# e4s2024/E4S2024

Hardware: AMD Instinct MI355X
Metric: 1024x1024 faces/sec (StyleGAN2 regional synthesis, gen_img) (higher is better)
Workload: dtype f16+mxfp6x2 (masked 3x3 layers >= 32^2) / bf16x3 (all other layers); 1 GPU; BASELINE configs[1]: StyleGAN2 1024x1024 synthesis from random W+, 12-region masks, batch=4/GPU; batch_per_gpu=4, global_batch=4, parallelism=frames x1, streams_per_gpu=2

## Files before the change

### e4s2024_amd/_lib.py

```python
from __future__ import annotations

import ctypes
import os
import re

HERE = os.path.dirname(os.path.abspath(__file__))
SO_PATH = os.environ.get("E4S_HIP_LIB") or os.path.join(HERE, "lib", "libe4s_hip.so")
HEADER = os.path.join(os.path.dirname(HERE), "include", "e4s_hip.h")

c_int, c_i64, c_f32, c_ptr = ctypes.c_int, ctypes.c_int64, ctypes.c_float, ctypes.c_void_p

_SCALARS = {"int": c_int, "int64_t": c_i64, "float": c_f32, "unsigned": ctypes.c_uint}
_RETURNS = {"int": c_int, "const char*": ctypes.c_char_p}


def _ctype(decl: str, where: str):
    if "*" in decl:
        return c_ptr
    ty = " ".join(decl.split()[:-1])
    if ty not in _SCALARS:
        raise TypeError(f"{where}: no ctypes rule for '{' '.join(decl.split())}' (known: pointers, {', '.join(_SCALARS)})")
    return _SCALARS[ty]


# ... 14 lines not shown
    for ret, name, args in re.findall(r"E4S_API\s+([\w\s*]+?)\s*\b(e4s_\w+)\s*\(([^()]*)\)\s*;", code):
        ret = " ".join(ret.split())
        if ret not in _RETURNS:
            raise TypeError(f"{name}: no ctypes rule for the return type '{ret}' (known: {', '.join(_RETURNS)})")
        restypes[name] = _RETURNS[ret]
        args = [] if args.strip() in ("", "void") else args.split(",")
        protos[name] = [_ctype(a, f"{name}: argument {i}") for i, a in enumerate(args)]
    if len(protos) != len(re.findall(r"\bE4S_API\b", code)):
        raise TypeError(f"the header has {len(re.findall('E4S_API', code))} E4S_API declarations, {len(protos)} were understood")
    return protos, restypes, structs, defines


with open(HEADER) as _f:
    _PROTOS, _RESTYPES, _STRUCTS, _DEFINES = parse_header(_f.read())

ABI_VERSION, ERR_ARG, MAX_REGIONS, LABEL_NONE, MAX_STYLE_JOBS, MAX_TARGETS, X_NHWC, OUT_NHWC, X_SP, OUT_SP = (_DEFINES["E4S_" + n] for n in (
    "ABI_VERSION", "ERR_ARG", "MAX_REGIONS", "LABEL_NONE", "MAX_STYLE_JOBS", "MAX_TARGETS", "X_NHWC", "OUT_NHWC", "X_SP", "OUT_SP"))


def targets(ptrs, weights):
    k = len(ptrs)
    if not 1 <= k <= MAX_TARGETS or len(weights) != k:
        raise ValueError(f"1 .. {MAX_TARGETS} targets with one weight each, got {k} targets and {len(weights)} weights")
    return (c_ptr * k)(*ptrs), (c_f32 * k)(*[float(w) for w in weights]), k


def declared_symbols():
    return list(_PROTOS)


class StyleJob(ctypes.Structure):
    _fields_ = _STRUCTS["E4sStyleJob"]
# ... 43 lines not shown
```

### e4s2024_amd/csrc/modconv_mx4.hip

```cpp
#include "modconv_mx_tile.h"

namespace {

constexpr int Q_TN = 64;
constexpr int Q_W1B = 3 * 2 * Q_TN * 16;
constexpr int Q_F6LO = 2 * 2 * Q_TN * 16;
constexpr int Q_F6HI = 2 * 2 * Q_TN * 8;
constexpr int Q_SCB = 1024;
constexpr int Q_PARB = Q_W1B + Q_F6LO + Q_F6HI + Q_SCB;
constexpr int Q_ROWB = 4 * Q_PARB;
constexpr int Q_NPIECE = Q_ROWB / 1024;
using CQ = SbCfg<2, 1, 1, 8, 5>;
constexpr int Q_PSTRIDE = 352;
constexpr int Q_PATCHB = 4 * Q_PSTRIDE * 16;
constexpr int Q_SSB = E4S_MAX_REGIONS * CKS * 4;
constexpr int Q_PATCH0 = 2 * Q_ROWB, Q_SS0 = Q_PATCH0 + 2 * Q_PATCHB, Q_LDS = Q_SS0 + 2 * Q_SSB;
static_assert(Q_LDS + 16 <= 160 * 1024 && (E4S_MAX_REGIONS + 1) * Q_TN * 4 <= Q_ROWB, "LDS plan");

#define Q_FENCE() do { asm volatile("" ::: "memory"); __builtin_amdgcn_sched_barrier(0); } while (0)

__global__ __launch_bounds__(256) void prep_weights_mx4_kernel(unsigned char* __restrict__ dst, const float* __restrict__ weight, const float* __restrict__ blur,
                                                               int cout, int cin, float scale) {
    const int nchunk = (cin + CKS - 1) / CKS;
    const int ntile = (cout + Q_TN - 1) / Q_TN;
// ... 265 lines not shown
    } else {
        c = l % G;
        item = l / G;
    }
    const int ntile = p.tiles_x * p.tiles_y;
    const int tile = (int)(item % (unsigned)ntile), b = (int)(item / (unsigned)ntile);
    const int y0 = (tile / p.tiles_x) * CQ::TH, x0 = (tile % p.tiles_x) * CQ::TW;
    int c_own;
    const bool uni = quad_uniform_tile(p, b, y0, x0, (int)(threadIdx.x >> 6), (int)(threadIdx.x & 31), c_own, reinterpret_cast<volatile int*>(lds_raw + Q_LDS));
    if (uni) {
        if (phase) return;
        q_tile_body(p, lds_raw, tile, (int)c, b, c_own);
    } else {
        SbParams pc = p;
        pc.wmx = reinterpret_cast<const unsigned char*>(p.whi);
        mx_tile_body<1, false, false, false>(pc, lds_raw, tile, (int)(2u * phase + (c & 1u)), 0, (int)(c >> 1), b);
    }
}

}

extern "C" int e4s_modconv_mx4_weight_bytes(int cout, int cin, int64_t* bytes) {
    E4S_REQUIRE(bytes && cout >= 1 && cin >= 1, "modconv_mx4_weight_bytes: bad arguments");
    *bytes = (int64_t)cdiv(cin, CKS) * cdiv(cout, Q_TN) * 3 * Q_ROWB;
    return 0;
}

extern "C" int e4s_modconv_prep_weights_mx4(void* dst, const float* weight, const float* blur, int cout, int cin, void* stream) {
    E4S_REQUIRE(dst && weight && blur, "modconv_prep_weights_mx4: null tensor");
    E4S_REQUIRE(cout >= 1 && cin >= 1, "modconv_prep_weights_mx4: bad size");
    E4S_REQUIRE(((uintptr_t)dst & 15) == 0, "modconv_prep_weights_mx4: the destination must be 16-byte aligned");
// ... 40 lines not shown
```

### e4s2024_amd/csrc/modconv_mx_tile.h

```cpp
#pragma once
#include <stdlib.h>

#include "common.h"
#include "sb_common.h"
#include "modconv_sb.h"

using namespace e4s;

#ifndef MX_ABL
#define MX_ABL 0
#endif

namespace {


typedef _Float16 f16x8 __attribute__((ext_vector_type(8)));
typedef _Float16 f16x2 __attribute__((ext_vector_type(2)));
typedef _Float16 f16x32 __attribute__((ext_vector_type(32)));
typedef unsigned u32x16 __attribute__((ext_vector_type(16)));
typedef unsigned u32x6 __attribute__((ext_vector_type(6)));
typedef int i32x8 __attribute__((ext_vector_type(8)));

constexpr int MX_TN = 128;
constexpr int MX_ROWB0 = 2 * 3 * 2 * MX_TN * 16;
// ... 78 lines not shown
struct MxLds {
    static constexpr int ROWB = ARITH ? MX_ROWB1 : MX_ROWB0;
    static constexpr int RING = 3 * ROWB;
    static constexpr int PATCH0 = RING;
    static constexpr int SS0 = PATCH0 + 2 * MX_PATCHB;
    static constexpr int BYTES = SS0 + 2 * MX_SSB;
    static constexpr int NPIECE = ROWB / 1024;
    static_assert(ROWB % 1024 == 0 && BYTES <= 160 * 1024, "LDS plan");
    static_assert((E4S_MAX_REGIONS + 5) * MX_TN * 4 + 64 <= RING, "the epilogue's tables overlay the weight ring");
};

constexpr int MX_NORM_MAX_CIN = 1024;
constexpr int MX_NORM_BYTES = 2 * MX_NORM_MAX_CIN * 4;
static_assert(MxLds<0>::BYTES + MX_NORM_BYTES <= 160 * 1024 && MxLds<1>::BYTES + MX_NORM_BYTES <= 160 * 1024, "LDS plan of the plain-convolution mode");

template <int ARITH, bool RGB, bool OSP, bool ENC = false>
__device__ __forceinline__ void mx_tile_body(const SbParams& p, unsigned char* lds_raw, const int tile, const int par, const int ks, const int cotile, const int b) {
    static_assert(!ENC || (!RGB && !OSP), "plain-convolution mode has its own epilogue");
    using L = MxLds<ARITH>;

    const int tid = threadIdx.x;
    const int lane = tid & 63;
    const int wave = __builtin_amdgcn_readfirstlane(tid >> 6) & 7;
    const int l5 = lane & 31, khalf = lane >> 5;

    const int pa = par >> 1, pb_ = par & 1;
    const int y0 = (tile / p.tiles_x) * C::TH, x0 = (tile % p.tiles_x) * C::TW;
    const int co0 = cotile * MX_TN;
    const int hw = p.h * p.w;
    const int ho = p.up ? 2 * p.h : p.h, wo = p.up ? 2 * p.w : p.w;
    const int nchunk = (p.cin + CKS - 1) / CKS;
// ... 344 lines not shown
                    if (co0 + n < p.cout) op[(size_t)(co0 + n) * hw] = v;
                }
        }
        return;
    }
    if (p.ksplit > 1) {
        float* part = p.partial + ((size_t)ks * p.bs + b) * p.cout * ho * wo;
        const int y = y0 + wave, x = x0 + l5;
        if (y < p.h && x < p.w) {
            const size_t opix = (size_t)(p.up ? 2 * y + pa : y) * wo + (p.up ? 2 * x + pb_ : x);
#pragma unroll
            for (int i = 0; i < 4; ++i)
#pragma unroll
                for (int r = 0; r < 16; ++r) {
                    const int co = co0 + i * 32 + (r & 3) + 8 * (r >> 2) + 4 * khalf;
                    if (co < p.cout) part[(size_t)co * ho * wo + opix] = acc[i][0][r];
                }
        }
        return;
    }
    if constexpr (MX_ABL & 1024) { if (acc[0][0][0] == 12345.f) p.out[tid] = acc[1][0][1] + acc[2][0][2] + acc[3][0][3]; return; }
    sb_epilogue<C, 4, 1, 8, RGB, OSP>(p, lds_raw, acc, cls, co0, b, y0, x0, pa, pb_, ho, wo, ub_skip);
}

}
```

### e4s2024_amd/csrc/modconv_sb.h

```cpp
#pragma once
#include "common.h"
#include "sb_common.h"

namespace e4s {

struct SbParams {
    float* out;
    const float* x;
    const uint4* whi;
    const uint4* wlo;
    const float* s;
    const float* d;
    const uint8_t* labels;
    const float* noise;
    const float* noise_weight;
    const float* act_bias;
    int lh, lw;
    float lscale_y, lscale_x;
    int noise_bstride;
    int act;
    int bs, cin, cout, h, w, nreg, up;
    int x_nhwc, out_nhwc;
    int tiles_x, tiles_y;
    int ksplit, chunks_per;
// ... 3 lines not shown
    const float* rgb_s;
    const float* rgb_bias;
    const float* rgb_skip;
    const float* rgb_upk;
    const float* s_next;
    int64_t plane_out;
    const uint8_t* uni_blocks;
    const int* uni_ctrl;
    const unsigned char* wmx;
    const float* in_mean;
    const float* in_rstd;
    const float* slope;
    int xcd_remap;
    int* flags;
    unsigned perm_mul;
};

template <int CB, int PB, int WC, int WP, int LOG_TW>
struct SbCfg {
    static constexpr int TN = WC * CB * 32;
    static constexpr int NPB = WP * PB;
    static constexpr int TW = 1 << LOG_TW;
    static constexpr int RPB = 32 >> LOG_TW;
    static constexpr int BPR = TW > 32 ? TW / 32 : 1;
    static constexpr int TH = TW > 32 ? NPB / BPR : NPB * RPB;
    static_assert(TW <= 32 || NPB % BPR == 0, "whole rows only");
    __host__ __device__ static constexpr int blk_y(int pbk, int l5) { return TW > 32 ? pbk / BPR : pbk * RPB + (l5 >> LOG_TW); }
    __host__ __device__ static constexpr int blk_x(int pbk, int l5) { return TW > 32 ? (pbk % BPR) * 32 + l5 : (l5 & (TW - 1)); }
    static constexpr int PW = TW + 2, PH = TH + 2;
    static constexpr int PATCH = PH * PW;
// ... 200 lines not shown
#pragma unroll
            for (int q = 0; q < PB; ++q) {
                const int pbk = wp * PB + q;
                const int y = y0 + C::blk_y(pbk, l5), x = x0 + C::blk_x(pbk, l5);
                if (y < p.h && x < p.w) {
                    const size_t opix = (size_t)y * wo + x;
#pragma unroll
                    for (int o = 0; o < 3; ++o)
                        p.rgb_out[((size_t)b * 3 + o) * ho * wo + opix] = rgbp[q][o] + xch[o * (C::NPB * 32) + pbk * 32 + l5] + rgbadd[q][o];
                }
            }
        }
    }
}

int launch_modconv_mx(SbParams& p, int arith, hipStream_t st, float* workspace, int64_t workspace_floats, bool plain_conv = false);

}
```

### e4s2024_amd/csrc/modconv_sb.hip

```cpp
#include <stdlib.h>

#include "common.h"
#include "sb_common.h"
#include "modconv_sb.h"

using namespace e4s;

__global__ __launch_bounds__(256) void prep_weights_sb_kernel(uint16_t* __restrict__ whi, uint16_t* __restrict__ wlo,
                                                              const float* __restrict__ weight, const float* __restrict__ blur, int cout,
                                                              int cin, int up, float scale) {
    const int npar = up ? 4 : 1;
    const int nchunk = (cin + CKS - 1) / CKS;
    const int64_t total = (int64_t)npar * nchunk * 9 * 2 * cout * 8;
    for (int64_t i = (int64_t)blockIdx.x * 256 + threadIdx.x; i < total; i += (int64_t)gridDim.x * 256) {
        const int e = (int)(i & 7);
        int64_t r = i >> 3;
        const int co = (int)(r % cout); r /= cout;
        const int half = (int)(r & 1); r >>= 1;
        const int tap = (int)(r % 9); r /= 9;
        const int chunk = (int)(r % nchunk);
        const int par = (int)(r / nchunk);
        const int ci = chunk * CKS + half * 8 + e;
        float v = 0.f;
        if (ci < cin) {
// ... 331 lines not shown
    }

    if (p.ksplit > 1) {
        float* part = p.partial + ((size_t)ks * p.bs + b) * p.cout * ho * wo;
#pragma unroll
        for (int q = 0; q < PB; ++q) {
            const int pbk = wp * PB + q;
            const int y = y0 + C::blk_y(pbk, l5), x = x0 + C::blk_x(pbk, l5);
            if (y >= p.h || x >= p.w) continue;
            const size_t opix = (size_t)(p.up ? 2 * y + pa : y) * wo + (p.up ? 2 * x + pb_ : x);
#pragma unroll
            for (int i = 0; i < CB; ++i)
#pragma unroll
                for (int r = 0; r < 16; ++r) {
                    const int co = co0 + (wc * CB + i) * 32 + (r & 3) + 8 * (r >> 2) + 4 * khalf;
                    if (co < p.cout) part[(size_t)co * ho * wo + opix] = acc[i][q][r];
                }
        }
        return;
    }

    E4S_PROF_MARK(g_prof_sb, 3);
    sb_epilogue<C, CB, PB, WP, RGB, OSP>(p, lds_raw, acc, cls, co0, b, y0, x0, pa, pb_, ho, wo, ub_skip);
    E4S_PROF_MARK(g_prof_sb, 4);
    E4S_PROF_DRAIN();
    E4S_PROF_MARK(g_prof_sb, 5);
}

__global__ __launch_bounds__(256) void modconv_sb_finalize_kernel(const SbParams p, int ho, int wo) {
    const size_t ohw = (size_t)ho * wo;
    const size_t per_b = (size_t)p.cout * ohw;
    const size_t total = (size_t)p.bs * per_b;
    const float nw = p.noise ? p.noise_weight[0] : 0.f;
    for (size_t i = (size_t)blockIdx.x * 256 + threadIdx.x; i < total; i += (size_t)gridDim.x * 256) {
        const int b = (int)(i / per_b);
        const size_t r = i - (size_t)b * per_b;
        const int co = (int)(r / ohw);
        const size_t opix = r - (size_t)co * ohw;
        const int oy = (int)(opix / wo), ox = (int)(opix - (size_t)oy * wo);
        float a = 0.f;
        for (int k = 0; k < p.ksplit; ++k) a += p.partial[(size_t)k * total + i];
        int c = 0;
        if (p.labels) c = p.labels[((size_t)b * p.lh + nearest_src(oy, p.lscale_y, p.lh)) * p.lw + nearest_src(ox, p.lscale_x, p.lw)];
        float v = 0.f;
        if (c < p.nreg) v = a * (p.d ? p.d[((size_t)b * p.nreg + c) * p.cout + co] : 1.f);
        if (p.noise) v += nw * p.noise[(size_t)b * p.noise_bstride + opix];
        if (p.act_bias) v += p.act_bias[co];
        if (p.act) v = (v > 0.f ? v : v * 0.2f) * 1.41421356237309515f;
        p.out[i] = v;
    }
}

template <int CB, int PB, int WC, int WP, int LOG_TW>
static int launch_sb_tconv(SbParams& p, hipStream_t st) {
    using C = SbCfg<CB, PB, WC, WP, LOG_TW>;
    p.tiles_x = cdiv(p.w + 1, C::TW);
    p.tiles_y = cdiv(p.h + 1, C::TH);
    p.up = 0;
    p.ksplit = 1;
    p.chunks_per = cdiv(p.cin, CKS);
    p.partial = nullptr;
    dim3 grid(p.tiles_x * p.tiles_y, cdiv(p.cout, C::TN), p.bs);
    hipLaunchKernelGGL((region_modconv_sb_kernel<CB, PB, WC, WP, LOG_TW, 2, true, true>), grid, dim3(C::NT), C::LDS_BYTES, st, p);
    return check_launch("modconv_tconv_sb");
// ... 57 lines not shown
    constexpr bool BIG = C::LDS_BYTES > 64 * 1024;
    constexpr int BIGW = C::NT / 256;
    if constexpr (BIG) {
        if (p.x_nhwc) return fail(E4S_ERR_ARG, "region_modconv3x3_sb: channels-last input is built for the single-region layers only");
        static const hipError_t attr = hipFuncSetAttribute(reinterpret_cast<const void*>(&region_modconv_sb_kernel<CB, PB, WC, WP, LOG_TW, BIGW, false, false>),
                                                           hipFuncAttributeMaxDynamicSharedMemorySize, C::LDS_BYTES);
        if (attr != hipSuccess) return fail((int)attr, "region_modconv3x3_sb: cannot raise the dynamic LDS limit: %s", hipGetErrorString(attr));
        hipLaunchKernelGGL((region_modconv_sb_kernel<CB, PB, WC, WP, LOG_TW, BIGW, false, false>), grid, dim3(C::NT), C::LDS_BYTES, st, p);
    } else if (p.x_nhwc) {
        if (p.labels || p.nreg != 1) return fail(E4S_ERR_ARG, "region_modconv3x3_sb: channels-last input is built for the single-region layers only");
        hipLaunchKernelGGL((region_modconv_sb_kernel<CB, PB, WC, WP, LOG_TW, 2, true, false, false, true>), grid, dim3(C::NT), uni_lds, st, p);
    } else if (!p.labels && p.nreg == 1)
        hipLaunchKernelGGL((region_modconv_sb_kernel<CB, PB, WC, WP, LOG_TW, 2, true, false>), grid, dim3(C::NT), uni_lds, st, p);
    else
        hipLaunchKernelGGL((region_modconv_sb_kernel<CB, PB, WC, WP, LOG_TW, 2, false, false>), grid, dim3(C::NT), C::LDS_BYTES, st, p);
    if (ksplit > 1) {
        const int g = (int)(cdiv64(out_floats, 256) < 2048 ? cdiv64(out_floats, 256) : 2048);
        hipLaunchKernelGGL(modconv_sb_finalize_kernel, dim3(g), dim3(256), 0, st, p, ho, wo);
    }
    return check_launch("region_modconv3x3_sb");
}

static inline bool layout_in_out_nhwc(int layout) { return (layout & (E4S_X_NHWC | E4S_OUT_NHWC)) != 0; }

static int region_modconv3x3_sb_impl(float* out, const float* x, const uint16_t* whi, const uint16_t* wlo, const float* s, const float* d,
                                     const uint8_t* labels, int lh, int lw, const float* noise, int noise_bs, const float* noise_weight,
                                     const float* act_bias, int act, int bs, int cin, int cout, int h, int w, int nreg, int up,
                                     float* workspace, int64_t workspace_floats, float* rgb_out, const float* rgb_wt, const float* rgb_s,
                                     const float* rgb_bias, const float* rgb_skip, const float* rgb_up_kernel, const float* s_next,
                                     const uint8_t* uniform_blocks, const int* uniform_ctrl, const void* wmx, int arith, int* flags, void* stream) {
    const int layout = up & (E4S_X_NHWC | E4S_OUT_NHWC | E4S_OUT_SP);
    up &= 1;
    const bool empty = bs == 0;
    E4S_REQUIRE(!(layout & E4S_OUT_SP) || (((s_next && rgb_out && out) || empty) && cout % 8 == 0 && !(layout & E4S_OUT_NHWC) && ((uintptr_t)out & 15) == 0),
                "region_modconv3x3_sb: split-plane output needs s_next, the fused ToRGB, cout %% 8 == 0 and a 16-byte aligned tensor");
    E4S_REQUIRE((((out || rgb_out) && x && s) || empty) && ((whi && wlo) || wmx), "region_modconv3x3_sb: null tensor");
    E4S_REQUIRE(!rgb_out || (rgb_wt && rgb_s && rgb_bias && (!rgb_skip || rgb_up_kernel) && w >= 32 && !up), "region_modconv3x3_sb: incomplete fused-ToRGB arguments");
    E4S_REQUIRE(bs >= 0 && cin >= 1 && cout >= 1 && h >= 1 && w >= 1, "region_modconv3x3_sb: bad size");
    E4S_REQUIRE(nreg >= 1 && nreg <= E4S_MAX_REGIONS, "region_modconv3x3_sb: %d regions (max %d)", nreg, E4S_MAX_REGIONS);
    E4S_REQUIRE(labels || nreg == 1 || empty, "region_modconv3x3_sb: nreg > 1 needs a label map");
    E4S_REQUIRE(!labels || (lh >= 1 && lw >= 1), "region_modconv3x3_sb: bad label map size");
    E4S_REQUIRE(!noise || (noise_weight && (noise_bs == 1 || noise_bs == bs)), "region_modconv3x3_sb: noise needs its weight and batch 1 or bs");
    E4S_REQUIRE(bs <= 65535, "region_modconv3x3_sb: batch too large");
    E4S_REQUIRE((((uintptr_t)whi | (uintptr_t)wlo) & 15) == 0, "region_modconv3x3_sb: weight slabs must be 16-byte aligned");
    if (bs == 0) return 0;
    SbParams p;
// ... 9 lines not shown
    const int ho = up ? 2 * h : h, wo = up ? 2 * w : w;
    p.lscale_y = labels ? (float)lh / (float)ho : 1.f;
    p.lscale_x = labels ? (float)lw / (float)wo : 1.f;
    p.noise_bstride = (noise && noise_bs > 1) ? ho * wo : 0;
    p.rgb_out = rgb_out; p.rgb_wt = rgb_wt; p.rgb_s = rgb_s; p.rgb_bias = rgb_bias; p.rgb_skip = rgb_skip; p.rgb_upk = rgb_up_kernel;
    p.s_next = (layout & E4S_OUT_SP) ? s_next : nullptr;
    p.plane_out = (int64_t)bs * (cout / 8) * ho * wo;
    E4S_REQUIRE(!uniform_blocks || (up && labels && w >= 32 && cout >= 128 && (h % 8) == 0 && (w % 8) == 0 && !layout),
                "region_modconv3x3_sb: the uniform-block map goes with a masked up layer of width >= 32, cout >= 128, h and w multiples of 8");
    E4S_REQUIRE(!uniform_blocks || uniform_ctrl, "region_modconv3x3_sb: the uniform-block map comes with its control words (e4s_uniform_blocks)");
    p.uni_blocks = uniform_blocks;
    p.uni_ctrl = uniform_ctrl;
    p.perm_mul = 0;
    p.wmx = reinterpret_cast<const unsigned char*>(wmx);
    p.flags = flags;
    hipStream_t st = (hipStream_t)stream;
    float* ws = p.out_nhwc ? nullptr : workspace;
    const int64_t wf = p.out_nhwc ? 0 : workspace_floats;
    if (wmx) {
        E4S_REQUIRE(labels && w >= 32 && cout >= 128 && cin % CKS == 0 && !layout_in_out_nhwc(layout) && ((uintptr_t)wmx & 15) == 0 && (arith == 0 || arith == 1),
                    "region_modconv3x3_mx: built for masked layers of width >= 32, cout >= 128, cin %% 16 == 0, channels-first activations");
        if (int rc = launch_modconv_mx(p, arith, st, ws, wf)) return rc;
        if (p.ksplit > 1) {
            const int64_t out_floats = (int64_t)bs * cout * ho * wo;
            const int g = (int)(cdiv64(out_floats, 256) < 2048 ? cdiv64(out_floats, 256) : 2048);
            hipLaunchKernelGGL(modconv_sb_finalize_kernel, dim3(g), dim3(256), 0, st, p, ho, wo);
            return check_launch("region_modconv3x3_mx");
        }
        return 0;
    }
    if (w >= 32) {
        constexpr int tw64 = 1;
        if (w >= 64 && !labels && (tw64 & 1) && !p.x_nhwc) {
            if (cout > 32) return launch_sb<2, 2, 1, 4, 6>(p, st, ws, wf);
            return launch_sb<1, 2, 1, 4, 6>(p, st, ws, wf);
        }
        if (w >= 64 && labels && cout >= 128 && (tw64 & 2)) return launch_sb<4, 1, 1, 8, 6>(p, st, ws, wf);
        if (labels && cout >= 128) return launch_sb<4, 1, 1, 8, 5>(p, st, ws, wf);
// ... 137 lines not shown
```

### e4s2024_amd/dropin/models/stylegan2/model.py

```python
import math
import random

import torch
from torch import nn

from e4s2024_amd import ops, torch_ref
from models.stylegan2.op import FusedLeakyReLU, fused_leaky_relu, upfirdn2d


class PixelNorm(nn.Module):

    def __init__(self):
        super().__init__()

    def forward(self, input):
        return input * torch.rsqrt(torch.mean(input ** 2, dim=1, keepdim=True) + 1e-8)


def make_kernel(k):
    k = torch.tensor(k, dtype=torch.float32)
    if k.ndim == 1:
        k = k[None, :] * k[:, None]
    k /= k.sum()
    return k
# ... 149 lines not shown
        saved = (s, d, self._weights(labels is not None)[1]) if labels is not None else None
        up_blocks = None
        if (self.upsample and labels is not None and ops.UP_BLOCKS and ops.MODCONV_MODE == "sb" and self.kernel_size == 3 and ops.mx_arith() == 1
                and input.shape[-1] >= max(32, ops.UP_BLOCKS_MIN_WIDTH) and self.out_channel >= 128 and self.in_channel % 32 == 0 and self.in_channel <= 512
                and not torch.is_grad_enabled()):
            up_blocks = (self._prepared_ubmx.get(self.weight, None, False, 7), self.blur.kernel)
        mx = mx4 = None
        if (self.kernel_size == 3 and not (x_nhwc or out_nhwc) and isinstance(wt, tuple)
                and ops.mx_eligible(self.in_channel, self.out_channel, input.shape[-1], labels is not None)):
            arith = ops.mx_arith()
            mx = (self._prepared_mx.get(self.weight, self.blur.kernel if self.upsample else None, self.upsample, arith), arith)
            if (self.upsample and arith == 1 and up_blocks is None and rgb is None
                    and ops.mx4_eligible(self.in_channel, self.out_channel, input.shape[-2], input.shape[-1], input.shape[0])):
                mx4 = self._prepared_mx4.get(self.weight, self.blur.kernel, True, 4)
        out = ops.region_modconv3x3(input, wt, s, d, labels, noise, noise_weight, act_bias, act, self.out_channel, self.upsample, rgb=rgb,
                                    want_out=want_out, x_nhwc=x_nhwc, out_nhwc=out_nhwc, s_next=s_next, up_blocks=up_blocks, mx=mx, mx4=mx4)
        if x_nhwc or out_nhwc or s_next is not None:
            return out
        if rgb is not None:
            return tuple(None if o is None else ops._attach("ModulatedConv2d", o, input, styles, self.weight, self.modulation.weight,
                                                            self.modulation.bias, noise_weight, act_bias) for o in out)
        return ops._attach("ModulatedConv2d", out, input, styles, self.weight, self.modulation.weight, self.modulation.bias, noise_weight,
                           act_bias, ref=self._torch_ref(labels, noise, act, saved))

    def _torch_ref(self, labels, noise, act, tables=None):
        blur = self.blur.kernel if self.upsample else None
        mod = self.modulation

        def ref(x, styles, weight, mod_w, mod_b, noise_weight, act_bias, fwd_out=None):
            return torch_ref.styled_conv(x, styles, weight, mod_w, mod_b, noise_weight, act_bias, labels=labels, noise=noise, act=act,
                                         upsample=self.upsample, blur=blur, demodulate=self.demodulate, mod_scale=mod.scale, mod_lr=mod.lr_mul,
# ... 339 lines not shown
```

### e4s2024_amd/ops.py

```python
from __future__ import annotations

import ctypes
import math
import os
import threading
import weakref
from typing import Optional, Sequence, Tuple

import torch

from ._lib import LABEL_NONE, MAX_REGIONS, MAX_STYLE_JOBS, OUT_NHWC, OUT_SP, X_NHWC, X_SP, ChainLayer, StyleJob, lib

SQRT2 = 2.0 ** 0.5


def _p(t: Optional[torch.Tensor]):
    return None if t is None else ctypes.c_void_p(t.data_ptr())


def _stream():
    return ctypes.c_void_p(torch.cuda.current_stream().cuda_stream)


def _req(t: torch.Tensor, name: str, dtype=torch.float32) -> torch.Tensor:
    if not isinstance(t, torch.Tensor):
        raise TypeError(f"{name} must be a torch.Tensor")
# ... 744 lines not shown
    cin = mw.shape[0]
    s = torch.empty((bs, nreg, cin), dtype=torch.float32, device=styles.device)
    d = torch.empty((bs, nreg, cout), dtype=torch.float32, device=styles.device) if wsq is not None else None
    lib().call("e4s_style_demod", _p(s), _p(d), _p(styles), styles.stride(0), styles.stride(1), _p(mw), _p(mb), _p(wsq), bs, nreg, cin, cout,
               sdim, _stream())
    return s, d


SPLITK_MAX_OUT_FLOATS = 1 << 21


def _workspace(device, floats: int) -> torch.Tensor:
    c = _ctx()
    ws = c.workspace
    if ws is None or ws.device != torch.device(device):
        ws = c.workspace = torch.empty(16 * SPLITK_MAX_OUT_FLOATS, dtype=torch.float32, device=device)
    if ws.numel() < floats:
        raise RuntimeError(f"split-K workspace request of {floats} floats exceeds its fixed size {ws.numel()}")
    return ws


NHWC_CHAIN = True
SP_CHAIN = os.environ.get("E4S_SP_CHAIN", "1") != "0"
NHWC_LINKS = "all"


def nhwc_link(kind: str, stage: int) -> bool:
    items = NHWC_LINKS.split(",")
    return NHWC_CHAIN and (NHWC_LINKS == "all" or kind in items or f"{kind}{stage}" in items)
FUSE_RGB = True


def can_fuse_rgb(cout: int, w: int, up: bool, masked: bool) -> bool:
# ... 16 lines not shown
    bs, lh, lw = lab.shape
    if ho % UP_BLOCK or wo % UP_BLOCK:
        raise ValueError("uniform_blocks: output size must be a multiple of 16")
    blocks = torch.empty((bs, ho // UP_BLOCK, wo // UP_BLOCK), dtype=torch.uint8, device=lab.device)
    sub = torch.empty((bs, ho // 8, wo // 8), dtype=torch.uint8, device=lab.device)
    ctx = _ctx()
    ctrl = getattr(ctx, "up_ctrl", None)
    if ctrl is None or ctrl.device != lab.device:
        ctrl = ctx.up_ctrl = torch.zeros((4,), dtype=torch.int32, device=lab.device)
    lib().call("e4s_uniform_blocks", _p(blocks), _p(sub), _p(ctrl), _p(lab), bs, lh, lw, ho, wo, nreg, 0,
               UP_BLOCKS_MIN_PERCENT if min_percent is None else int(min_percent), _stream())
    return (blocks, sub, ctrl) if with_ctrl else (blocks, sub)


def region_modconv3x3(x, wt, s, d, labels, noise, noise_weight, act_bias, act: bool, cout: int, up: bool, rgb=None, want_out: bool = True,
                      x_nhwc: bool = False, out_nhwc: bool = False, s_next=None, up_blocks=None, mx=None, mx4=None):
    x = _c(x, "input")
    if x_nhwc:
        bs, cb, h, w, _ = x.shape
        cin = cb * 8
    else:
        bs, cin, h, w = x.shape
    nreg = s.shape[1]
    ho, wo = (2 * h, 2 * w) if up else (h, w)
    if not want_out and rgb is None:
        raise ValueError("want_out=False only makes sense together with a fused ToRGB")
    if (x_nhwc or out_nhwc) and not (isinstance(wt, tuple) and w >= 32 and cin % 16 == 0 and cout % 8 == 0):
        raise ValueError("channel-blocked activations need the split-bf16 kernel, width >= 32, cin % 16 == 0 and cout % 8 == 0")
    sn = None
    if s_next is not None:
        if rgb is None or not want_out or out_nhwc or up or cout % 8:
# ... 6 lines not shown
    if labels is not None:
        lh, lw = labels.shape[1:]
        if labels.shape[0] != bs:
            raise ValueError(f"mask batch {labels.shape[0]} != input batch {bs}")
    nz = nbs = None
    if noise is not None:
        nz = _c(noise, "noise")
        nbs = nz.shape[0]
        if nz.numel() != nbs * ho * wo:
            raise ValueError(f"noise shape {tuple(nz.shape)} does not match output {ho}x{wo}")
    ws, wsn = None, 0
    if bs * cout * ho * wo <= SPLITK_MAX_OUT_FLOATS and sn is None:
        wsn = 16 * bs * cout * ho * wo
        ws = _workspace(x.device, wsn)
    sb = isinstance(wt, tuple)
    blocks = bctrl = None
    if (up_blocks is not None and UP_BLOCKS and sb and up and labels is not None and mx is not None and mx[1] == 1 and w >= max(32, UP_BLOCKS_MIN_WIDTH) and cout >= 128
            and h % 8 == 0 and w % 16 == 0 and cin % 32 == 0 and cin <= 512 and rgb is None and not (x_nhwc or out_nhwc) and sn is None):
        wmx_blocks, blur_k = up_blocks
        composed_wgs = (wo // 64) * (ho // 16) * 4 * -(-cout // 128) * bs
        blocks, sub, bctrl = uniform_blocks(labels, ho, wo, nreg, with_ctrl=True,
                                            min_percent=max(UP_BLOCKS_MIN_PERCENT, UP_BLOCKS_MIN_PERCENT_SMALL) if composed_wgs <= 512 else UP_BLOCKS_MIN_PERCENT)
        if UP_BLOCKS_ONLY_ONE_KERNEL is not None:
            out.fill_(float("nan"))
        evb = _timed("masked_upconv_blocks", f"{cin}->{cout} @{h} up")
        if UP_BLOCKS_ONLY_ONE_KERNEL != "composed":
            lib().call("e4s_masked_upconv_blocks_mx", _p(out), _p(x), _p(wmx_blocks), _p(mx_flags(x.device)), _p(s), _p(d), _p(blocks), _p(bctrl), _p(_c(blur_k, "blur kernel")),
                       _p(nz), nbs or 0, _p(noise_weight) if nz is not None else None, _p(act_bias), 1 if act else 0, bs, cin, cout, h, w, nreg, _stream())
        if evb is not None:
            evb.record()
# ... 10 lines not shown
            raise ValueError(f"skip shape {tuple(r_skip.shape)} != {(bs, 3, ho // 2, wo // 2)}")
        rgb_args = (_p(rgb_out), _p(r_wt), _p(r_s), _p(_c(r_bias.detach(), "bias")), _p(_c(r_skip, "skip")) if r_skip is not None else None,
                    _p(_c(r_upk, "upsample.kernel")) if r_skip is not None else None)
    else:
        rgb_args = (None,) * 6
    if sb and mx is not None:
        if labels is None or w < 32 or cout < 128 or cin % 16 or x_nhwc or out_nhwc:
            raise ValueError("region_modconv3x3: the mx kernel is built for masked layers of width >= 32, cout >= 128, cin % 16 == 0, channels-first")
        wmx, arith = mx
        if mx4 is not None and up and arith == 1 and blocks is None and rgb is None and sn is None and cout % 128 == 0:
            lib().call("e4s_region_upconv_mx4", _p(out), _p(x), _p(mx4), _p(wmx), _p(mx_flags(x.device)), _p(s), _p(d), _p(labels), lh, lw, _p(nz), nbs or 0,
                       _p(noise_weight) if nz is not None else None, _p(act_bias), 1 if act else 0, bs, cin, cout, h, w, nreg, _stream())
        else:
            lib().call("e4s_region_modconv3x3_mx", _p(out), _p(x), _p(wmx), arith, _p(mx_flags(x.device)) if arith else None, _p(s), _p(d), _p(labels), lh, lw,
                       _p(nz), nbs or 0, _p(noise_weight) if nz is not None else None, _p(act_bias), 1 if act else 0, bs, cin, cout, h, w, nreg,
                       (1 if up else 0) | (OUT_SP if sn is not None else 0), _p(ws), wsn, *rgb_args, _p(sn),
                       _p(blocks), _p(bctrl) if blocks is not None else None, _stream())
    elif sb:
        lib().call("e4s_region_modconv3x3_sb", _p(out), _p(x), _p(wt[0]), _p(wt[1]), _p(s), _p(d), _p(labels), lh, lw, _p(nz), nbs or 0,
                   _p(noise_weight) if nz is not None else None, _p(act_bias), 1 if act else 0, bs, cin, cout, h, w, nreg,
                   (1 if up else 0) | (X_NHWC if x_nhwc else 0) | (OUT_NHWC if out_nhwc else 0) | (OUT_SP if sn is not None else 0), _p(ws), wsn, *rgb_args, _p(sn),
                   _p(blocks), _p(bctrl) if blocks is not None else None, _stream())
    else:
        lib().call("e4s_region_modconv3x3", _p(out), _p(x), _p(wt), _p(s), _p(d), _p(labels), lh, lw, _p(nz), nbs or 0,
                   _p(noise_weight) if nz is not None else None, _p(act_bias), 1 if act else 0, bs, cin, cout, h, w, nreg, 1 if up else 0,
                   _p(ws), wsn, _stream())
    if ev is not None:
        ev.record()
    return out if rgb is None else (out, rgb_out)


def _alloc_split_planes(bs: int, c: int, h: int, w: int, device) -> torch.Tensor:
    n = 2 * bs * c * h * w
    return torch.empty(n + 8, dtype=torch.int16, device=device)[:n].view(2, bs, c // 8, h, w, 8)


# ... 234 lines not shown
```

### include/e4s_hip.h

```cpp
#ifndef E4S_HIP_H
#define E4S_HIP_H

#include <stdint.h>

#ifdef __cplusplus
extern "C" {
#endif

#define E4S_API __attribute__((visibility("default")))
#define E4S_ABI_VERSION 1
#define E4S_ERR_ARG (-1)
#define E4S_MAX_REGIONS 16
#define E4S_LABEL_NONE 255

E4S_API int e4s_abi_version(void);
E4S_API const char* e4s_last_error(void);

E4S_API int e4s_fused_bias_act(float* out, const float* x, const float* bias, const float* ref,
                       int act, int grad, float alpha, float scale,
                       int64_t size_x, int64_t step_b, int64_t size_b, void* stream);

E4S_API int e4s_upfirdn2d(float* out, const float* in, const float* kernel,
                  int major, int in_h, int in_w, int kh, int kw,
                  int up_x, int up_y, int down_x, int down_y,
// ... 22 lines not shown
} E4sStyleJob;
E4S_API int e4s_style_demod_batched(const E4sStyleJob* jobs, int n_jobs, int bs, int sdim, void* stream);

E4S_API int e4s_region_modconv3x3(float* out, const float* x, const float* wt, const float* s, const float* d,
                          const uint8_t* labels, int lh, int lw,
                          const float* noise, int noise_bs, const float* noise_weight, const float* act_bias, int act,
                          int bs, int cin, int cout, int h, int w, int nreg, int up,
                          float* workspace, int64_t workspace_floats, void* stream);

E4S_API int e4s_modconv_prep_weights_sb(uint16_t* whi, uint16_t* wlo, float* wsq, const float* weight, const float* blur,
                                        int cout, int cin, int up, void* stream);
#define E4S_X_NHWC 2
#define E4S_OUT_NHWC 4
#define E4S_X_SP 8
#define E4S_OUT_SP 16
E4S_API int e4s_region_modconv3x3_sb(float* out, const float* x, const uint16_t* whi, const uint16_t* wlo, const float* s, const float* d,
                                     const uint8_t* labels, int lh, int lw,
                                     const float* noise, int noise_bs, const float* noise_weight, const float* act_bias, int act,
                                     int bs, int cin, int cout, int h, int w, int nreg, int up,
                                     float* workspace, int64_t workspace_floats,
                                     float* rgb_out, const float* rgb_wt, const float* rgb_s, const float* rgb_bias,
                                     const float* rgb_skip, const float* rgb_up_kernel, const float* s_next,
                                     const uint8_t* uniform_blocks, const int* uniform_ctrl, void* stream);

E4S_API int e4s_modconv_mx_weight_bytes(int cout, int cin, int up, int arith, int64_t* bytes);
E4S_API int e4s_modconv_prep_weights_mx(void* dst, const float* weight, const float* blur, int cout, int cin, int up, int arith, void* stream);
E4S_API int e4s_region_modconv3x3_mx(float* out, const float* x, const void* wmx, int arith, int* flags, const float* s, const float* d,
                                     const uint8_t* labels, int lh, int lw,
                                     const float* noise, int noise_bs, const float* noise_weight, const float* act_bias, int act,
                                     int bs, int cin, int cout, int h, int w, int nreg, int up,
// ... 390 lines not shown
```

Baseline: 1581 faces/s.

## Fuse split-K reduction into the conv kernel via last-arriver tile counters

Split-K modulated-conv launches now keep a per-tile arrival counter in the workspace tail. The last block to finish a tile sums the partials and applies the demod/noise/bias/activation epilogue, so the separate finalize kernel launch is skipped. This removes one kernel launch and one full pass over the partial buffer per split-K layer. In exchange, partial stores become agent-scope atomic stores and every block pays for an extra barrier and a counter atomic, and the reduction work falls to a single block per tile.

```diff
diff --git a/e4s2024_amd/_lib.py b/e4s2024_amd/_lib.py
--- a/e4s2024_amd/_lib.py
+++ b/e4s2024_amd/_lib.py
@@ -52,8 +52,8 @@
 with open(HEADER) as _f:
     _PROTOS, _RESTYPES, _STRUCTS, _DEFINES = parse_header(_f.read())
 
-ABI_VERSION, ERR_ARG, MAX_REGIONS, LABEL_NONE, MAX_STYLE_JOBS, MAX_TARGETS, X_NHWC, OUT_NHWC, X_SP, OUT_SP = (_DEFINES["E4S_" + n] for n in (
-    "ABI_VERSION", "ERR_ARG", "MAX_REGIONS", "LABEL_NONE", "MAX_STYLE_JOBS", "MAX_TARGETS", "X_NHWC", "OUT_NHWC", "X_SP", "OUT_SP"))
+ABI_VERSION, ERR_ARG, MAX_REGIONS, LABEL_NONE, MAX_STYLE_JOBS, MAX_TARGETS, X_NHWC, OUT_NHWC, X_SP, OUT_SP, WS_COUNTERS, SPLITK_COUNTERS = (_DEFINES["E4S_" + n] for n in (
+    "ABI_VERSION", "ERR_ARG", "MAX_REGIONS", "LABEL_NONE", "MAX_STYLE_JOBS", "MAX_TARGETS", "X_NHWC", "OUT_NHWC", "X_SP", "OUT_SP", "WS_COUNTERS", "SPLITK_COUNTERS"))
 
 
 def targets(ptrs, weights):
diff --git a/e4s2024_amd/csrc/modconv_mx4.hip b/e4s2024_amd/csrc/modconv_mx4.hip
--- a/e4s2024_amd/csrc/modconv_mx4.hip
+++ b/e4s2024_amd/csrc/modconv_mx4.hip
@@ -303,7 +303,7 @@
     } else {
         SbParams pc = p;
         pc.wmx = reinterpret_cast<const unsigned char*>(p.whi);
-        mx_tile_body<1, false, false, false>(pc, lds_raw, tile, (int)(2u * phase + (c & 1u)), 0, (int)(c >> 1), b);
+        mx_tile_body<1, false, false, false, false>(pc, lds_raw, tile, (int)(2u * phase + (c & 1u)), 0, (int)(c >> 1), b);
     }
 }
 
diff --git a/e4s2024_amd/csrc/modconv_mx_tile.h b/e4s2024_amd/csrc/modconv_mx_tile.h
--- a/e4s2024_amd/csrc/modconv_mx_tile.h
+++ b/e4s2024_amd/csrc/modconv_mx_tile.h
@@ -116,7 +116,7 @@
 constexpr int MX_NORM_BYTES = 2 * MX_NORM_MAX_CIN * 4;
 static_assert(MxLds<0>::BYTES + MX_NORM_BYTES <= 160 * 1024 && MxLds<1>::BYTES + MX_NORM_BYTES <= 160 * 1024, "LDS plan of the plain-convolution mode");
 
-template <int ARITH, bool RGB, bool OSP, bool ENC = false>
+template <int ARITH, bool RGB, bool OSP, bool ENC = false, bool SPLITK = true>
 __device__ __forceinline__ void mx_tile_body(const SbParams& p, unsigned char* lds_raw, const int tile, const int par, const int ks, const int cotile, const int b) {
     static_assert(!ENC || (!RGB && !OSP), "plain-convolution mode has its own epilogue");
     using L = MxLds<ARITH>;
@@ -491,9 +491,14 @@
 #pragma unroll
                 for (int r = 0; r < 16; ++r) {
                     const int co = co0 + i * 32 + (r & 3) + 8 * (r >> 2) + 4 * khalf;
-                    if (co < p.cout) part[(size_t)co * ho * wo + opix] = acc[i][0][r];
-                }
-        }
+                    if (co < p.cout) splitk_store(part + (size_t)co * ho * wo + opix, acc[i][0][r], SPLITK && p.splitk_ctr != nullptr);
+                }
+        }
+        if (RGB || OSP || !SPLITK || !p.splitk_ctr) return;
+        const int npar = p.up ? 4 : 1;
+        int* ctr = p.splitk_ctr + (((size_t)b * ncot + cotile) * npar + par) * (p.tiles_x * p.tiles_y) + tile;
+        if (splitk_last_arriver(ctr, p.ksplit, reinterpret_cast<volatile int*>(lds_raw)))
+            splitk_reduce_tile<C, 4, 1, 8>(p, cls, co0, b, y0, x0, pa, pb_, ho, wo);
         return;
     }
     if constexpr (MX_ABL & 1024) { if (acc[0][0][0] == 12345.f) p.out[tid] = acc[1][0][1] + acc[2][0][2] + acc[3][0][3]; return; }
diff --git a/e4s2024_amd/csrc/modconv_sb.h b/e4s2024_amd/csrc/modconv_sb.h
--- a/e4s2024_amd/csrc/modconv_sb.h
+++ b/e4s2024_amd/csrc/modconv_sb.h
@@ -41,6 +41,7 @@
     int xcd_remap;
     int* flags;
     unsigned perm_mul;
+    int* splitk_ctr;
 };
 
 template <int CB, int PB, int WC, int WP, int LOG_TW>
@@ -271,6 +272,81 @@
     }
 }
 
+__device__ __forceinline__ float splitk_epilogue(float a, bool in_region, float d, bool has_noise, float nw, float nz, bool has_bias, float bias, int act) {
+    float v = 0.f;
+    if (in_region) v = __fmul_rn(a, d);
+    if (has_noise) v = __fmaf_rn(nw, nz, v);
+    if (has_bias) v = __fadd_rn(v, bias);
+    if (act) v = __fmul_rn(v > 0.f ? v : __fmul_rn(v, 0.2f), 1.41421356237309515f);
+    return v;
+}
+
+__device__ __forceinline__ void splitk_store(float* dst, float v, bool through) {
+    if (through) __hip_atomic_store(dst, v, __ATOMIC_RELAXED, __HIP_MEMORY_SCOPE_AGENT);
+    else *dst = v;
+}
+
+__device__ __forceinline__ bool splitk_last_arriver(int* ctr, int ksplit, volatile int* flagw) {
+    asm volatile("s_waitcnt vmcnt(0)" ::: "memory");
+    __syncthreads();
+    if (threadIdx.x == 0) {
+        const int ticket = __hip_atomic_fetch_add(ctr, 1, __ATOMIC_RELAXED, __HIP_MEMORY_SCOPE_AGENT);
+        const bool last = ticket == ksplit - 1;
+        if (last) {
+            __hip_atomic_store(ctr, 0, __ATOMIC_RELAXED, __HIP_MEMORY_SCOPE_AGENT);
+            __builtin_amdgcn_fence(__ATOMIC_ACQUIRE, "agent");
+            asm volatile("s_waitcnt vmcnt(0)" ::: "memory");
+        }
+        *flagw = last ? 1 : 0;
+    }
+    __syncthreads();
+    return *flagw != 0;
+}
+
+template <class C, int CB, int PB, int WP>
+__device__ __forceinline__ void splitk_reduce_tile(const SbParams& p, const int (&cls)[PB], int co0, int b, int y0, int x0, int pa, int pb_, int ho, int wo) {
+    const int lane = threadIdx.x & 63, wave = threadIdx.x >> 6;
+    const int l5 = lane & 31, khalf = lane >> 5;
+    const int wc = wave / WP, wp = wave % WP;
+    const size_t ohw = (size_t)ho * wo;
+    const size_t slice = (size_t)p.bs * p.cout * ohw;
+    const float* part = p.partial + (size_t)b * p.cout * ohw;
+    float* outb = p.out + (size_t)b * p.cout * ohw;
+    const bool has_noise = p.noise != nullptr, has_bias = p.act_bias != nullptr;
+    const float nw = has_noise ? p.noise_weight[0] : 0.f;
+#pragma unroll
+    for (int q = 0; q < PB; ++q) {
+        const int pbk = wp * PB + q;
+        const int y = y0 + C::blk_y(pbk, l5), x = x0 + C::blk_x(pbk, l5);
+        if (y >= p.h || x >= p.w) continue;
+        const size_t opix = (size_t)(p.up ? 2 * y + pa : y) * wo + (p.up ? 2 * x + pb_ : x);
+        const float nz = has_noise ? p.noise[(size_t)b * p.noise_bstride + opix] : 0.f;
+        const bool in_region = cls[q] >= 0;
+        const float* drow = (p.d && in_region) ? p.d + ((size_t)b * p.nreg + cls[q]) * p.cout : nullptr;
+#pragma unroll
+        for (int i = 0; i < CB; ++i) {
+            const int cb0 = co0 + (wc * CB + i) * 32 + 4 * khalf;
+            float a[16];
+#pragma unroll
+            for (int r = 0; r < 16; ++r) a[r] = 0.f;
+            for (int k = 0; k < p.ksplit; ++k) {
+                const float* pk = part + (size_t)k * slice + opix;
+#pragma unroll
+                for (int r = 0; r < 16; ++r) {
+                    const int co = cb0 + (r & 3) + 8 * (r >> 2);
+                    if (co < p.cout) a[r] += pk[(size_t)co * ohw];
+                }
+            }
+#pragma unroll
+            for (int r = 0; r < 16; ++r) {
+                const int co = cb0 + (r & 3) + 8 * (r >> 2);
+                if (co < p.cout)
+                    outb[(size_t)co * ohw + opix] = splitk_epilogue(a[r], in_region, drow ? drow[co] : 1.f, has_noise, nw, nz, has_bias, has_bias ? p.act_bias[co] : 0.f, p.act);
+            }
+        }
+    }
+}
+
 int launch_modconv_mx(SbParams& p, int arith, hipStream_t st, float* workspace, int64_t workspace_floats, bool plain_conv = false);
 
 }
diff --git a/e4s2024_amd/csrc/modconv_sb.hip b/e4s2024_amd/csrc/modconv_sb.hip
--- a/e4s2024_amd/csrc/modconv_sb.hip
+++ b/e4s2024_amd/csrc/modconv_sb.hip
@@ -369,9 +369,13 @@
 #pragma unroll
                 for (int r = 0; r < 16; ++r) {
                     const int co = co0 + (wc * CB + i) * 32 + (r & 3) + 8 * (r >> 2) + 4 * khalf;
-                    if (co < p.cout) part[(size_t)co * ho * wo + opix] = acc[i][q][r];
+                    if (co < p.cout) splitk_store(part + (size_t)co * ho * wo + opix, acc[i][q][r], p.splitk_ctr != nullptr);
                 }
         }
+        if (RGB || OSP || !p.splitk_ctr) return;
+        int* ctr = p.splitk_ctr + (((size_t)b * gridDim.y + blockIdx.y) * npar + par) * ntile + tile;
+        if (splitk_last_arriver(ctr, p.ksplit, reinterpret_cast<volatile int*>(lds_raw)))
+            splitk_reduce_tile<C, CB, PB, WP>(p, cls, co0, b, y0, x0, pa, pb_, ho, wo);
         return;
     }
 
@@ -397,12 +401,9 @@
         for (int k = 0; k < p.ksplit; ++k) a += p.partial[(size_t)k * total + i];
         int c = 0;
         if (p.labels) c = p.labels[((size_t)b * p.lh + nearest_src(oy, p.lscale_y, p.lh)) * p.lw + nearest_src(ox, p.lscale_x, p.lw)];
-        float v = 0.f;
-        if (c < p.nreg) v = a * (p.d ? p.d[((size_t)b * p.nreg + c) * p.cout + co] : 1.f);
-        if (p.noise) v += nw * p.noise[(size_t)b * p.noise_bstride + opix];
-        if (p.act_bias) v += p.act_bias[co];
-        if (p.act) v = (v > 0.f ? v : v * 0.2f) * 1.41421356237309515f;
-        p.out[i] = v;
+        const bool in_region = c < p.nreg;
+        p.out[i] = splitk_epilogue(a, in_region, (p.d && in_region) ? p.d[((size_t)b * p.nreg + c) * p.cout + co] : 1.f, p.noise != nullptr, nw,
+                                   p.noise ? p.noise[(size_t)b * p.noise_bstride + opix] : 0.f, p.act_bias != nullptr, p.act_bias ? p.act_bias[co] : 0.f, p.act);
     }
 }
 
@@ -490,7 +491,7 @@
         hipLaunchKernelGGL((region_modconv_sb_kernel<CB, PB, WC, WP, LOG_TW, 2, true, false>), grid, dim3(C::NT), uni_lds, st, p);
     else
         hipLaunchKernelGGL((region_modconv_sb_kernel<CB, PB, WC, WP, LOG_TW, 2, false, false>), grid, dim3(C::NT), C::LDS_BYTES, st, p);
-    if (ksplit > 1) {
+    if (ksplit > 1 && !p.splitk_ctr) {
         const int g = (int)(cdiv64(out_floats, 256) < 2048 ? cdiv64(out_floats, 256) : 2048);
         hipLaunchKernelGGL(modconv_sb_finalize_kernel, dim3(g), dim3(256), 0, st, p, ho, wo);
     }
@@ -506,6 +507,13 @@
                                      const float* rgb_bias, const float* rgb_skip, const float* rgb_up_kernel, const float* s_next,
                                      const uint8_t* uniform_blocks, const int* uniform_ctrl, const void* wmx, int arith, int* flags, void* stream) {
     const int layout = up & (E4S_X_NHWC | E4S_OUT_NHWC | E4S_OUT_SP);
+    static_assert(E4S_SPLITK_COUNTERS >= 384, "one counter per tile of a K-split launch");
+    int* counters = nullptr;
+    if (up & E4S_WS_COUNTERS) {
+        E4S_REQUIRE(workspace && workspace_floats > E4S_SPLITK_COUNTERS, "region_modconv3x3_sb: E4S_WS_COUNTERS needs a workspace of more than %d floats", E4S_SPLITK_COUNTERS);
+        workspace_floats -= E4S_SPLITK_COUNTERS;
+        counters = reinterpret_cast<int*>(workspace + workspace_floats);
+    }
     up &= 1;
     const bool empty = bs == 0;
     E4S_REQUIRE(!(layout & E4S_OUT_SP) || (((s_next && rgb_out && out) || empty) && cout % 8 == 0 && !(layout & E4S_OUT_NHWC) && ((uintptr_t)out & 15) == 0),
@@ -545,6 +553,7 @@
     p.perm_mul = 0;
     p.wmx = reinterpret_cast<const unsigned char*>(wmx);
     p.flags = flags;
+    p.splitk_ctr = counters;
     hipStream_t st = (hipStream_t)stream;
     float* ws = p.out_nhwc ? nullptr : workspace;
     const int64_t wf = p.out_nhwc ? 0 : workspace_floats;
@@ -552,7 +561,7 @@
         E4S_REQUIRE(labels && w >= 32 && cout >= 128 && cin % CKS == 0 && !layout_in_out_nhwc(layout) && ((uintptr_t)wmx & 15) == 0 && (arith == 0 || arith == 1),
                     "region_modconv3x3_mx: built for masked layers of width >= 32, cout >= 128, cin %% 16 == 0, channels-first activations");
         if (int rc = launch_modconv_mx(p, arith, st, ws, wf)) return rc;
-        if (p.ksplit > 1) {
+        if (p.ksplit > 1 && !p.splitk_ctr) {
             const int64_t out_floats = (int64_t)bs * cout * ho * wo;
             const int g = (int)(cdiv64(out_floats, 256) < 2048 ? cdiv64(out_floats, 256) : 2048);
             hipLaunchKernelGGL(modconv_sb_finalize_kernel, dim3(g), dim3(256), 0, st, p, ho, wo);
diff --git a/e4s2024_amd/dropin/models/stylegan2/model.py b/e4s2024_amd/dropin/models/stylegan2/model.py
--- a/e4s2024_amd/dropin/models/stylegan2/model.py
+++ b/e4s2024_amd/dropin/models/stylegan2/model.py
@@ -187,7 +187,7 @@
                     and ops.mx4_eligible(self.in_channel, self.out_channel, input.shape[-2], input.shape[-1], input.shape[0])):
                 mx4 = self._prepared_mx4.get(self.weight, self.blur.kernel, True, 4)
         out = ops.region_modconv3x3(input, wt, s, d, labels, noise, noise_weight, act_bias, act, self.out_channel, self.upsample, rgb=rgb,
-                                    want_out=want_out, x_nhwc=x_nhwc, out_nhwc=out_nhwc, s_next=s_next, up_blocks=up_blocks, mx=mx, mx4=mx4)
+                                    want_out=want_out, x_nhwc=x_nhwc, out_nhwc=out_nhwc, s_next=s_next, up_blocks=up_blocks, mx=mx, mx4=mx4, splitk_in_kernel=True)
         if x_nhwc or out_nhwc or s_next is not None:
             return out
         if rgb is not None:
diff --git a/e4s2024_amd/ops.py b/e4s2024_amd/ops.py
--- a/e4s2024_amd/ops.py
+++ b/e4s2024_amd/ops.py
@@ -9,7 +9,7 @@
 
 import torch
 
-from ._lib import LABEL_NONE, MAX_REGIONS, MAX_STYLE_JOBS, OUT_NHWC, OUT_SP, X_NHWC, X_SP, ChainLayer, StyleJob, lib
+from ._lib import LABEL_NONE, MAX_REGIONS, MAX_STYLE_JOBS, OUT_NHWC, OUT_SP, SPLITK_COUNTERS, WS_COUNTERS, X_NHWC, X_SP, ChainLayer, StyleJob, lib
 
 SQRT2 = 2.0 ** 0.5
 
@@ -784,9 +784,10 @@
     c = _ctx()
     ws = c.workspace
     if ws is None or ws.device != torch.device(device):
-        ws = c.workspace = torch.empty(16 * SPLITK_MAX_OUT_FLOATS, dtype=torch.float32, device=device)
-    if ws.numel() < floats:
-        raise RuntimeError(f"split-K workspace request of {floats} floats exceeds its fixed size {ws.numel()}")
+        ws = c.workspace = torch.empty(16 * SPLITK_MAX_OUT_FLOATS + SPLITK_COUNTERS, dtype=torch.float32, device=device)
+        ws[-SPLITK_COUNTERS:].zero_()
+    if ws.numel() - SPLITK_COUNTERS < floats:
+        raise RuntimeError(f"split-K workspace request of {floats} floats exceeds its fixed size {ws.numel() - SPLITK_COUNTERS}")
     return ws
 
 
@@ -833,7 +834,7 @@
 
 
 def region_modconv3x3(x, wt, s, d, labels, noise, noise_weight, act_bias, act: bool, cout: int, up: bool, rgb=None, want_out: bool = True,
-                      x_nhwc: bool = False, out_nhwc: bool = False, s_next=None, up_blocks=None, mx=None, mx4=None):
+                      x_nhwc: bool = False, out_nhwc: bool = False, s_next=None, up_blocks=None, mx=None, mx4=None, splitk_in_kernel: bool = False):
     x = _c(x, "input")
     if x_nhwc:
         bs, cb, h, w, _ = x.shape
@@ -870,6 +871,9 @@
         wsn = 16 * bs * cout * ho * wo
         ws = _workspace(x.device, wsn)
     sb = isinstance(wt, tuple)
+    ctr = 0
+    if splitk_in_kernel and sb and ws is not None:
+        ctr, wsn = WS_COUNTERS, ws.numel()
     blocks = bctrl = None
     if (up_blocks is not None and UP_BLOCKS and sb and up and labels is not None and mx is not None and mx[1] == 1 and w >= max(32, UP_BLOCKS_MIN_WIDTH) and cout >= 128
             and h % 8 == 0 and w % 16 == 0 and cin % 32 == 0 and cin <= 512 and rgb is None and not (x_nhwc or out_nhwc) and sn is None):
@@ -910,12 +914,12 @@
         else:
             lib().call("e4s_region_modconv3x3_mx", _p(out), _p(x), _p(wmx), arith, _p(mx_flags(x.device)) if arith else None, _p(s), _p(d), _p(labels), lh, lw,
                        _p(nz), nbs or 0, _p(noise_weight) if nz is not None else None, _p(act_bias), 1 if act else 0, bs, cin, cout, h, w, nreg,
-                       (1 if up else 0) | (OUT_SP if sn is not None else 0), _p(ws), wsn, *rgb_args, _p(sn),
+                       (1 if up else 0) | (OUT_SP if sn is not None else 0) | ctr, _p(ws), wsn, *rgb_args, _p(sn),
                        _p(blocks), _p(bctrl) if blocks is not None else None, _stream())
     elif sb:
         lib().call("e4s_region_modconv3x3_sb", _p(out), _p(x), _p(wt[0]), _p(wt[1]), _p(s), _p(d), _p(labels), lh, lw, _p(nz), nbs or 0,
                    _p(noise_weight) if nz is not None else None, _p(act_bias), 1 if act else 0, bs, cin, cout, h, w, nreg,
-                   (1 if up else 0) | (X_NHWC if x_nhwc else 0) | (OUT_NHWC if out_nhwc else 0) | (OUT_SP if sn is not None else 0), _p(ws), wsn, *rgb_args, _p(sn),
+                   (1 if up else 0) | (X_NHWC if x_nhwc else 0) | (OUT_NHWC if out_nhwc else 0) | (OUT_SP if sn is not None else 0) | ctr, _p(ws), wsn, *rgb_args, _p(sn),
                    _p(blocks), _p(bctrl) if blocks is not None else None, _stream())
     else:
         lib().call("e4s_region_modconv3x3", _p(out), _p(x), _p(wt), _p(s), _p(d), _p(labels), lh, lw, _p(nz), nbs or 0,
diff --git a/include/e4s_hip.h b/include/e4s_hip.h
--- a/include/e4s_hip.h
+++ b/include/e4s_hip.h
@@ -60,6 +60,8 @@
 #define E4S_OUT_NHWC 4
 #define E4S_X_SP 8
 #define E4S_OUT_SP 16
+#define E4S_WS_COUNTERS 32
+#define E4S_SPLITK_COUNTERS 384
 E4S_API int e4s_region_modconv3x3_sb(float* out, const float* x, const uint16_t* whi, const uint16_t* wlo, const float* s, const float* d,
                                      const uint8_t* labels, int lh, int lw,
                                      const float* noise, int noise_bs, const float* noise_weight, const float* act_bias, int act,
```

Result: slower. 1389 faces/s (-12.1%).
